# basilevh/occlusions-4d

Hardware: AMD Instinct MI355X
Metric: 4D query-points/sec (encode+decode) at n_points=14336 (higher is better)
Workload: dtype f32; 1 GPU; GREATER inference (BASELINE configs[1]): n_points=14336 video_len=12 num_sample=524288 (-> 534528 grid queries) implicit_batch_size=32768 (decoded in mini-batches of 32256 = 3584 workgroups of 9 queries; every query is decoded, results do not depend on the split), seeded random-init weights; abstract_points=531, outputs_per_query=5, parallelism=single GPU, schedule=sequential, rccl_ranks=1, decode_streams=2, decode_chunk=32256

## Files before the change

### occlusions-4d_amd/csrc/fps_bucket.hip

```cpp
#include "common.hpp"

#include <cstdlib>

namespace {

typedef unsigned long long u64;
typedef float f32x2 __attribute__((ext_vector_type(2)));

constexpr int FLAG_WORDS = 512;
constexpr int IDX_BITS = 14;
constexpr unsigned IDX_MASK = (1u << IDX_BITS) - 1u;

template <int OP>
__device__ __forceinline__ int wave_reduce(int v) {
#define OCC4D_DPP_STEP(ctrl)                                                                      \
  if (OP == 0) asm volatile("s_nop 1\n\tv_min_u32_dpp %0, %0, %0 " ctrl : "+v"(v));               \
  else asm volatile("s_nop 1\n\tv_max_i32_dpp %0, %0, %0 " ctrl : "+v"(v));
  OCC4D_DPP_STEP("quad_perm:[1,0,3,2] row_mask:0xf bank_mask:0xf")
  OCC4D_DPP_STEP("quad_perm:[2,3,0,1] row_mask:0xf bank_mask:0xf")
  OCC4D_DPP_STEP("row_half_mirror row_mask:0xf bank_mask:0xf")
  OCC4D_DPP_STEP("row_mirror row_mask:0xf bank_mask:0xf")
  OCC4D_DPP_STEP("row_bcast:15 row_mask:0xa bank_mask:0xf")
  OCC4D_DPP_STEP("row_bcast:31 row_mask:0xc bank_mask:0xf")
#undef OCC4D_DPP_STEP
  return __builtin_amdgcn_readlane(v, 63);
}

template <bool IS_MAX>
__device__ __forceinline__ float wave_reduce_f32(float v) {
#define OCC4D_DPP_STEP(ctrl)                                                                      \
  if (IS_MAX) asm volatile("s_nop 1\n\tv_max_f32_dpp %0, %0, %0 " ctrl : "+v"(v));               \
  else asm volatile("s_nop 1\n\tv_min_f32_dpp %0, %0, %0 " ctrl : "+v"(v));
  OCC4D_DPP_STEP("quad_perm:[1,0,3,2] row_mask:0xf bank_mask:0xf")
  OCC4D_DPP_STEP("quad_perm:[2,3,0,1] row_mask:0xf bank_mask:0xf")
  OCC4D_DPP_STEP("row_half_mirror row_mask:0xf bank_mask:0xf")
  OCC4D_DPP_STEP("row_mirror row_mask:0xf bank_mask:0xf")
  OCC4D_DPP_STEP("row_bcast:15 row_mask:0xa bank_mask:0xf")
  OCC4D_DPP_STEP("row_bcast:31 row_mask:0xc bank_mask:0xf")
#undef OCC4D_DPP_STEP
  return __int_as_float(__builtin_amdgcn_readlane(__float_as_int(v), 63));
}

template <typename E, int VL> struct vec_of { typedef E type __attribute__((ext_vector_type(VL))); };
constexpr int tuple_len(int len) { return len <= 2 ? 2 : len <= 4 ? 4 : len <= 8 ? 8 : len <= 16 ? 16 : 32; }

__device__ __forceinline__ unsigned spread3(unsigned x) {
  x = (x | (x << 8)) & 0x0300Fu;
  x = (x | (x << 4)) & 0x030C3u;
  x = (x | (x << 2)) & 0x09249u;
  return x;
}

__device__ __forceinline__ float block_reduce(float v, bool is_max, float* s_red, int t, int nw) {
  for (int o = 32; o > 0; o >>= 1) {
    const float w = __shfl_xor(v, o);
    v = is_max ? fmaxf(v, w) : fminf(v, w);
  }
  __syncthreads();
  if ((t & 63) == 0) s_red[t >> 6] = v;
  __syncthreads();
  float r = s_red[0];
  for (int w = 1; w < nw; ++w) r = is_max ? fmaxf(r, s_red[w]) : fminf(r, s_red[w]);
  return r;
}

template <int NB, int T>
__global__ __launch_bounds__(T) void fps_bucket_kernel(const float* __restrict__ xyz, int64_t stride, int n, int m,
                                                       int start, int32_t* __restrict__ out_sorted,
                                                       int32_t* __restrict__ out_order) {
  static_assert(NB >= 1 && NB <= 8, "buckets per wave: at most 8 (32 slots per lane)");
  constexpr int NW = T / 64;
  static_assert(NW == 8, "the candidate round below keeps candidate l % 8 in lane l");
  constexpr int CMAX = 8;
  constexpr int REFRESH = 8;
  constexpr int SORT_MAX = 16384;
  constexpr int CELL_BITS = 4, CELLS = 1 << (3 * CELL_BITS);
  static_assert(CELLS == 8 * T, "the scan below gives every thread eight cells");
  __shared__ unsigned short s_sort[SORT_MAX];
  __shared__ unsigned s_tmp[SORT_MAX];
  __shared__ unsigned s_hist[CELLS];
  __shared__ unsigned s_wsum[NW];
  __shared__ u64 s_key[2][NW];
  __shared__ float4 s_c[2][NW];
  __shared__ unsigned s_flags[FLAG_WORDS];
  __shared__ int s_cnt[T];
  __shared__ float s_red[NW];

  const int t = threadIdx.x;
  const int wave = t >> 6, lane = t & 63;

  float lo[3] = {__builtin_inff(), __builtin_inff(), __builtin_inff()};
  float hi[3] = {-__builtin_inff(), -__builtin_inff(), -__builtin_inff()};
  for (int i = t; i < n; i += T) {
    const float* p = xyz + (int64_t)i * stride;
#pragma unroll
    for (int a = 0; a < 3; ++a) {
      lo[a] = fminf(lo[a], p[a]);
      hi[a] = fmaxf(hi[a], p[a]);
    }
  }
  float scale[3];
#pragma unroll
  for (int a = 0; a < 3; ++a) {
    lo[a] = block_reduce(lo[a], false, s_red, t, NW);
    hi[a] = block_reduce(hi[a], true, s_red, t, NW);
    const float ext = hi[a] - lo[a];
    scale[a] = ext > 0.f ? (float)(1 << CELL_BITS) / ext : 0.f;
  }
  for (int c = t; c < CELLS; c += T) s_hist[c] = 0u;
  __syncthreads();
  for (int i = t; i < n; i += T) {
    const float* p = xyz + (int64_t)i * stride;
    unsigned cell = 0u;
#pragma unroll
    for (int a = 0; a < 3; ++a) {
      const int q = max(0, min((1 << CELL_BITS) - 1, (int)((p[a] - lo[a]) * scale[a])));
      cell |= spread3((unsigned)q) << a;
    }
    const unsigned rank = atomicAdd(&s_hist[cell], 1u);
    s_tmp[i] = (cell << IDX_BITS) | rank;
  }
  __syncthreads();
  {
    unsigned cnt[8], sum = 0u;
#pragma unroll
    for (int k = 0; k < 8; ++k) {
      cnt[k] = s_hist[8 * t + k];
      sum += cnt[k];
    }
    unsigned incl = sum;
    for (int o = 1; o < 64; o <<= 1) {
      const unsigned up = __shfl_up(incl, o);
      if (lane >= o) incl += up;
    }
    if (lane == 63) s_wsum[wave] = incl;
    __syncthreads();
    unsigned base = incl - sum;
    for (int w = 0; w < wave; ++w) base += s_wsum[w];
#pragma unroll
    for (int k = 0; k < 8; ++k) {
      s_hist[8 * t + k] = base;
      base += cnt[k];
    }
  }
  __syncthreads();
  for (int i = t; i < n; i += T) {
    const unsigned cr = s_tmp[i];
    s_sort[s_hist[cr >> IDX_BITS] + (cr & IDX_MASK)] = (unsigned short)i;
  }
  __syncthreads();

  constexpr int PPT = 4 * NB;
  typedef typename vec_of<float, tuple_len(PPT)>::type fvec;
  typedef typename vec_of<int, tuple_len(PPT)>::type ivec;
  typedef typename vec_of<int, tuple_len(2 * NB)>::type idvec;
  fvec px, py, pz;
  ivec md;
  idvec id;
  float bminx = 0.f, bminy = 0.f, bminz = 0.f, bmaxx = 0.f, bmaxy = 0.f, bmaxz = 0.f, bm = -1.f;
  const unsigned last = s_sort[n - 1];
#pragma clang loop unroll(disable)
  for (int u = 0; u < NB; ++u) {
    const int pos = ((u * NW + wave) << 8) + 4 * lane;
    float c[4][3], d0[4];
    unsigned ids[2] = {0u, 0u};
#pragma unroll
    for (int v = 0; v < 4; ++v) {
      const bool live = pos + v < n;
      const unsigned i = live ? (unsigned)s_sort[pos + v] : last;
      const float* p = xyz + (int64_t)i * stride;
      c[v][0] = p[0]; c[v][1] = p[1]; c[v][2] = p[2];
      d0[v] = live ? __builtin_inff() : -1.f;
      ids[v >> 1] |= (live ? i : 0xffffu) << (16 * (v & 1));
    }
    float bl[3], bh[3];
#pragma unroll
    for (int v = 0; v < 4; ++v) {
      px[4 * u + v] = c[v][0]; py[4 * u + v] = c[v][1]; pz[4 * u + v] = c[v][2];
      md[4 * u + v] = __float_as_int(d0[v]);
    }
    asm volatile("" : "+v"(ids[0]), "+v"(ids[1]));
    id[2 * u] = (int)ids[0]; id[2 * u + 1] = (int)ids[1];
#pragma unroll
    for (int a = 0; a < 3; ++a) {
      bl[a] = wave_reduce_f32<false>(fminf(fminf(c[0][a], c[1][a]), fminf(c[2][a], c[3][a])));
      bh[a] = wave_reduce_f32<true>(fmaxf(fmaxf(c[0][a], c[1][a]), fmaxf(c[2][a], c[3][a])));
    }
    const bool any_live = ((u * NW + wave) << 8) < n;
    if ((lane & 7) == u) {
      bminx = bl[0]; bminy = bl[1]; bminz = bl[2];
      bmaxx = bh[0]; bmaxy = bh[1]; bmaxz = bh[2];
      bm = any_live ? __builtin_inff() : -1.f;
    }
  }
  for (int w = t; w < FLAG_WORDS; w += T) s_flags[w] = 0u;
  __syncthreads();
  int gm[NB];
#pragma unroll
  for (int g = 0; g < NB; ++g) gm[g] = max(max(md[4 * g], md[4 * g + 1]), max(md[4 * g + 2], md[4 * g + 3]));
  const float* first = xyz + (int64_t)start * stride;
  float ccx = first[0], ccy = first[1], ccz = first[2];
  int nacc = 1;
  if (t == 0) {
    out_sorted[0] = start;
    if (out_order) out_order[0] = start;
  }

#ifdef OCC4D_FPSB_STAMP
  unsigned long long tacc[9] = {0, 0, 0, 0, 0, 0, 0, 0, 0};
  unsigned long long tprev = __builtin_amdgcn_s_memtime();
#define STAMP(i) { const unsigned long long tn = __builtin_amdgcn_s_memtime(); tacc[i] += tn - tprev; tprev = tn; }
#else
#define STAMP(i)
#endif
#define OCC4D_DPP8(op, v)                                                                          \
  asm volatile("s_nop 1\n\t" op " %0, %0, %0 quad_perm:[1,0,3,2] row_mask:0xf bank_mask:0xf\n\t"   \
               "s_nop 1\n\t" op " %0, %0, %0 quad_perm:[2,3,0,1] row_mask:0xf bank_mask:0xf\n\t"   \
               "s_nop 1\n\t" op " %0, %0, %0 row_half_mirror row_mask:0xf bank_mask:0xf" : "+v"(v))
  int par = 0, round = 0;
  for (int it = 1; it < m;) {
    if (round != 0 && (round & (REFRESH - 1)) == 0) {
#pragma unroll
      for (int u = 0; u < NB; ++u) {
        const int top = wave_reduce<1>(gm[u]);
        bm = (lane & 7) == u ? __int_as_float(top) : bm;
      }
    }
    ++round;
    const float ex = fmaxf(fmaxf(bminx - ccx, ccx - bmaxx), 0.f);
    const float ey = fmaxf(fmaxf(bminy - ccy, ccy - bmaxy), 0.f);
    const float ez = fmaxf(fmaxf(bminz - ccz, ccz - bmaxz), 0.f);
    const float db = (ex * ex + ey * ey) + ez * ez;
    const u64 touch = __ballot(db < bm && (lane >> 3) < nacc);
    STAMP(0)
#pragma unroll
    for (int u = 0; u < NB; ++u) {
      u64 mu = (touch >> u) & 0x0101010101010101ull;
      if (mu) {
        do {
          const int src = (int)__builtin_ctzll(mu) ;
          mu &= mu - 1;
          const float cx = __int_as_float(__builtin_amdgcn_readlane(__float_as_int(ccx), src));
          const float cy = __int_as_float(__builtin_amdgcn_readlane(__float_as_int(ccy), src));
          const float cz = __int_as_float(__builtin_amdgcn_readlane(__float_as_int(ccz), src));
          const f32x2 c2x = {cx, cx}, c2y = {cy, cy}, c2z = {cz, cz};
#pragma unroll
          for (int e = 4 * u; e < 4 * u + 4; e += 2) {
            const f32x2 dx = f32x2{px[e], px[e + 1]} - c2x;
            const f32x2 dy = f32x2{py[e], py[e + 1]} - c2y;
            const f32x2 dz = f32x2{pz[e], pz[e + 1]} - c2z;
            const f32x2 d = (dx * dx + dy * dy) + dz * dz;
            md[e] = min(__float_as_int(d[0]), md[e]);
            md[e + 1] = min(__float_as_int(d[1]), md[e + 1]);
          }
        } while (mu);
        gm[u] = max(max(md[4 * u], md[4 * u + 1]), max(md[4 * u + 2], md[4 * u + 3]));
      }
    }
    STAMP(1)
    int bd = gm[0];
#pragma unroll
    for (int g = 1; g < NB; ++g) bd = max(bd, gm[g]);
    const int wtop = wave_reduce<1>(bd);
    STAMP(2)
    constexpr int NEG1 = (int)0xbf800000;
    int hgroup = 0, lane_hits = 0, og = NEG1, sn = NEG1;
#pragma unroll
    for (int g = NB - 1; g >= 0; --g) {
      const bool e = gm[g] == wtop;
      hgroup = __ballot(e) ? g : hgroup;
      lane_hits += e ? 1 : 0;
      og = max(og, e ? NEG1 : gm[g]);
    }
    unsigned long long hit = 0ull;
    int hslot = 0, slot_hits = 0;
#pragma unroll
    for (int sl = 3; sl >= 0; --sl) {
      const int slot = hgroup * 4 + sl;
      const int v = md[slot];
      const bool e = v == wtop;
      const unsigned long long mk = __ballot(e);
      hit = mk ? mk : hit;
      hslot = mk ? slot : hslot;
      slot_hits += e ? 1 : 0;
      sn = max(sn, e ? NEG1 : v);
    }
    const bool single = __popcll(__ballot(lane_hits != 0)) == 1 && __ballot(lane_hits > 1 || slot_hits > 1) == 0ull;
    int hlane = (int)__builtin_ctzll(hit | (1ull << 63));
    unsigned widx;
    int wfloor = wtop;
    if (wtop >= 0 && !single) {
      unsigned cand = 0xffffffffu;
      int cslot = 0;
#pragma unroll
      for (int sl = 0; sl < PPT; ++sl) {
        const unsigned ids = (sl & 1) ? ((unsigned)id[sl >> 1] >> 16) : ((unsigned)id[sl >> 1] & 0xffffu);
        const bool better = md[sl] == wtop && ids < cand;
        cand = better ? ids : cand;
        cslot = better ? sl : cslot;
      }
      widx = (unsigned)wave_reduce<0>((int)cand);
      hlane = (int)__builtin_ctzll(__ballot(cand == widx) | (1ull << 63));
      hslot = __builtin_amdgcn_readlane(cslot, hlane);
    } else {
      const unsigned pair = (unsigned)__builtin_amdgcn_readlane(id[hslot >> 1], hlane);
      widx = (hslot & 1) ? (pair >> 16) : (pair & 0xffffu);
      if (wtop >= 0) wfloor = wave_reduce<1>(max(og, sn));
    }
    const float wx = __int_as_float(__builtin_amdgcn_readlane(__float_as_int(px[hslot]), hlane));
    const float wy = __int_as_float(__builtin_amdgcn_readlane(__float_as_int(py[hslot]), hlane));
    const float wz = __int_as_float(__builtin_amdgcn_readlane(__float_as_int(pz[hslot]), hlane));
    STAMP(3)
    if (lane == 0) {
      s_key[par][wave] = ((u64)(unsigned)max(wtop + 1, 0) << 32) |
                         (u64)(((IDX_MASK << 8) | (unsigned)wave) - ((widx & IDX_MASK) << 8));
      s_c[par][wave] = float4{wx, wy, wz, __int_as_float(wfloor)};
    }
    __syncthreads();
    STAMP(4)
    const int ci = lane & (NW - 1), ck = lane >> 3;
    const u64 key = s_key[par][ci];
    const float4 mine = s_c[par][ci], oth = s_c[par][ck];
    constexpr int TAKEN = (int)0x80000000, FAR = 0x7fffffff;
    const int khi = (int)(unsigned)(key >> 32);
    int cmd = khi ? khi - 1 : TAKEN;
    const int cidx = (int)(IDX_MASK - (((unsigned)key >> 8) & IDX_MASK));
    int fl = __float_as_int(mine.w);
    OCC4D_DPP8("v_max_i32_dpp", fl);
    const int F = __builtin_amdgcn_readfirstlane(fl);
    int D;
    {
      const float dx = mine.x - oth.x, dy = mine.y - oth.y, dz = mine.z - oth.z;
      D = __float_as_int((dx * dx + dy * dy) + dz * dz);
    }
    STAMP(5)
    const int room = min(CMAX, m - it);
    unsigned alist = 0u;
    int nnew = 0;
#pragma unroll
    for (int j = 0; j < CMAX; ++j) {
      int best = cmd;
      OCC4D_DPP8("v_max_i32_dpp", best);
      bool eq = cmd == best;
      unsigned m8 = (unsigned)__ballot(eq) & 0xffu;
      if (j == 0) {
        int low = eq ? cidx : FAR;
        OCC4D_DPP8("v_min_i32_dpp", low);
        eq = eq && cidx == low;
        m8 = (unsigned)__ballot(eq) & 0xffu;
      } else if (j >= room || !(__builtin_amdgcn_readfirstlane(best) > F) || (m8 & (m8 - 1u)) != 0u) {
        break;
      }
      const int a = __builtin_ctz(m8);
      alist |= (unsigned)a << (4 * j);
      nnew = j + 1;
      if (j == CMAX - 1) break;
      int red = ck == a ? D : FAR;
      asm volatile("s_nop 1\n\tv_min_i32_dpp %0, %0, %0 row_ror:8 row_mask:0xf bank_mask:0xf" : "+v"(red));
      {
        const auto r16 = __builtin_amdgcn_permlane16_swap((unsigned)red, (unsigned)red, false, false);
        red = min((int)r16[0], (int)r16[1]);
        const auto r32 = __builtin_amdgcn_permlane32_swap((unsigned)red, (unsigned)red, false, false);
        red = min((int)r32[0], (int)r32[1]);
      }
      cmd = eq ? TAKEN : min(cmd, red);
    }
    STAMP(6)
    {
      const int asel = (int)((alist >> (4 * ck)) & 7u);
      const float4 acc = s_c[par][asel];
      ccx = acc.x; ccy = acc.y; ccz = acc.z;
      if (wave == 0 && ci == 0 && ck < nnew) {
        const unsigned gi = IDX_MASK - (((unsigned)s_key[par][asel] >> 8) & IDX_MASK);
        const unsigned g = min(gi, (unsigned)(n - 1));
        out_sorted[it + ck] = (int)g;
        if (out_order) out_order[it + ck] = (int)g;
      }
    }
    nacc = nnew;
    it += nnew;
    STAMP(7)
    par ^= 1;
  }
#undef OCC4D_DPP8
  __syncthreads();
#ifdef OCC4D_FPSB_STAMP
  if (lane == 0 && out_order) {
    unsigned long long* o = (unsigned long long*)(out_order + ((m + 1) & ~1)) + wave * 16;
    tacc[8] = (unsigned long long)round;
#pragma unroll
    for (int i = 0; i < 9; ++i) o[i] = tacc[i];
  }
#endif

  for (int i = t; i < m; i += T) {
    const unsigned g = (unsigned)out_sorted[i];
    atomicOr(&s_flags[g >> 5], 1u << (g & 31));
  }
  __syncthreads();
  constexpr int CH = FLAG_WORDS / T;
  static_assert(CH >= 1, "T <= FLAG_WORDS");
  int cnt = 0;
#pragma unroll
  for (int c = 0; c < CH; ++c) cnt += __popc(s_flags[t * CH + c]);
  s_cnt[t] = cnt;
  __syncthreads();
  if (t == 0) {
    int run = 0;
    for (int i = 0; i < T; ++i) {
      const int c = s_cnt[i];
      s_cnt[i] = run;
      run += c;
    }
  }
  __syncthreads();
  int pos = s_cnt[t];
#pragma unroll
  for (int c = 0; c < CH; ++c) {
    unsigned wbits = s_flags[t * CH + c];
    while (wbits) {
      const int b = __ffs(wbits) - 1;
      wbits &= wbits - 1;
      if (pos < m) out_sorted[pos] = (t * CH + c) * 32 + b;
      ++pos;
    }
  }
}

}

namespace occ4d {

int fps_bucket_launch(const float* xyz, int64_t stride, int n, int m, int start, int32_t* os, int32_t* oo,
                      hipStream_t st) {
  static const int min_points = [] { const char* e = getenv("OCC4D_FPS_BUCKET_MIN"); return e ? atoi(e) : FPS_BUCKET_MIN_POINTS; }();
  if (n < min_points || n > 16384) return -1;
  constexpr int T = 512;
  const int nb = cdiv(n, 256 * (T / 64));
#define OCC4D_FPSB(B) fps_bucket_kernel<B, T><<<1, T, 0, st>>>(xyz, stride, n, m, start, os, oo)
  if (nb <= 1) OCC4D_FPSB(1);
  else if (nb <= 2) OCC4D_FPSB(2);
  else if (nb <= 3) OCC4D_FPSB(3);
  else if (nb <= 4) OCC4D_FPSB(4);
  else if (nb <= 5) OCC4D_FPSB(5);
  else if (nb <= 6) OCC4D_FPSB(6);
  else if (nb <= 7) OCC4D_FPSB(7);
  else OCC4D_FPSB(8);
#undef OCC4D_FPSB
  return 0;
}

}
```

Before: 4.651 million query-points/s.

## Propose two FPS candidates per wave to accept more points per round

Each wave in the bucketed farthest-point-sampling kernel now proposes its second-best point in addition to its best, giving 16 candidates per round. Wave 0 runs the greedy acceptance over all 16 with 16-lane DPP reductions and a 4-way distance table, then shares the accepted list through shared memory and an extra barrier. The aim is to accept more points per round and so cut the number of serial rounds and block-wide syncs. In exchange each round does more per-wave reduction work, adds a second __syncthreads, and leaves waves 1-7 idle during acceptance. The new path is the default, and OCC4D_FPS_CANDIDATES=1 restores the old one.

```diff
diff --git a/occlusions-4d_amd/csrc/fps_bucket.hip b/occlusions-4d_amd/csrc/fps_bucket.hip
--- a/occlusions-4d_amd/csrc/fps_bucket.hip
+++ b/occlusions-4d_amd/csrc/fps_bucket.hip
@@ -64,13 +64,15 @@
   return r;
 }
 
-template <int NB, int T>
+template <int NB, int T, int NC>
 __global__ __launch_bounds__(T) void fps_bucket_kernel(const float* __restrict__ xyz, int64_t stride, int n, int m,
                                                        int start, int32_t* __restrict__ out_sorted,
                                                        int32_t* __restrict__ out_order) {
   static_assert(NB >= 1 && NB <= 8, "buckets per wave: at most 8 (32 slots per lane)");
   constexpr int NW = T / 64;
-  static_assert(NW == 8, "the candidate round below keeps candidate l % 8 in lane l");
+  static_assert(NW == 8, "the candidate round below keeps candidate l % 8 (NC = 2: l % 16) in lane l");
+  static_assert(NC == 1 || NC == 2, "candidates per wave");
+  constexpr int NCAND = NC * NW;
   constexpr int CMAX = 8;
   constexpr int REFRESH = 8;
   constexpr int SORT_MAX = 16384;
@@ -80,8 +82,9 @@
   __shared__ unsigned s_tmp[SORT_MAX];
   __shared__ unsigned s_hist[CELLS];
   __shared__ unsigned s_wsum[NW];
-  __shared__ u64 s_key[2][NW];
-  __shared__ float4 s_c[2][NW];
+  __shared__ u64 s_key[2][NCAND];
+  __shared__ float4 s_c[2][NCAND];
+  __shared__ uint2 s_acc[2];
   __shared__ unsigned s_flags[FLAG_WORDS];
   __shared__ int s_cnt[T];
   __shared__ float s_red[NW];
@@ -217,6 +220,11 @@
   asm volatile("s_nop 1\n\t" op " %0, %0, %0 quad_perm:[1,0,3,2] row_mask:0xf bank_mask:0xf\n\t"   \
                "s_nop 1\n\t" op " %0, %0, %0 quad_perm:[2,3,0,1] row_mask:0xf bank_mask:0xf\n\t"   \
                "s_nop 1\n\t" op " %0, %0, %0 row_half_mirror row_mask:0xf bank_mask:0xf" : "+v"(v))
+#define OCC4D_DPP16(op, v)                                                                         \
+  asm volatile("s_nop 1\n\t" op " %0, %0, %0 quad_perm:[1,0,3,2] row_mask:0xf bank_mask:0xf\n\t"   \
+               "s_nop 1\n\t" op " %0, %0, %0 quad_perm:[2,3,0,1] row_mask:0xf bank_mask:0xf\n\t"   \
+               "s_nop 1\n\t" op " %0, %0, %0 row_half_mirror row_mask:0xf bank_mask:0xf\n\t"       \
+               "s_nop 1\n\t" op " %0, %0, %0 row_mirror row_mask:0xf bank_mask:0xf" : "+v"(v))
   int par = 0, round = 0;
   for (int it = 1; it < m;) {
     if (round != 0 && (round & (REFRESH - 1)) == 0) {
@@ -310,64 +318,169 @@
     const float wx = __int_as_float(__builtin_amdgcn_readlane(__float_as_int(px[hslot]), hlane));
     const float wy = __int_as_float(__builtin_amdgcn_readlane(__float_as_int(py[hslot]), hlane));
     const float wz = __int_as_float(__builtin_amdgcn_readlane(__float_as_int(pz[hslot]), hlane));
+    int w2 = NEG1;
+    unsigned widx2 = 0u;
+    float rx = 0.f, ry = 0.f, rz = 0.f;
+    if constexpr (NC == 2) {
+      if (single && wfloor >= 0) {
+        w2 = wfloor;
+        const bool wl = lane == hlane;
+        int hgroup2 = 0, group_hits2 = 0, og2 = NEG1, sn2 = NEG1;
+#pragma unroll
+        for (int g = NB - 1; g >= 0; --g) {
+          const int v = (wl && hgroup == g) ? sn : gm[g];
+          const bool e = v == w2;
+          const unsigned long long mk = __ballot(e);
+          hgroup2 = mk ? g : hgroup2;
+          group_hits2 += __popcll(mk);
+          og2 = max(og2, e ? NEG1 : v);
+        }
+        unsigned long long hit2 = 0ull;
+        int hslot2 = 0, slot_hits2 = 0;
+#pragma unroll
+        for (int sl = 3; sl >= 0; --sl) {
+          const int slot = hgroup2 * 4 + sl;
+          const int v = (wl && slot == hslot) ? NEG1 : md[slot];
+          const bool e = v == w2;
+          const unsigned long long mk = __ballot(e);
+          hit2 = mk ? mk : hit2;
+          hslot2 = mk ? slot : hslot2;
+          slot_hits2 += __popcll(mk);
+          sn2 = max(sn2, e ? NEG1 : v);
+        }
+        const bool single2 = group_hits2 == 1 && slot_hits2 == 1;
+        const int hlane2 = (int)__builtin_ctzll(hit2 | (1ull << 63));
+        const unsigned pair = (unsigned)__builtin_amdgcn_readlane(id[hslot2 >> 1], hlane2);
+        widx2 = (hslot2 & 1) ? (pair >> 16) : (pair & 0xffffu);
+        rx = __int_as_float(__builtin_amdgcn_readlane(__float_as_int(px[hslot2]), hlane2));
+        ry = __int_as_float(__builtin_amdgcn_readlane(__float_as_int(py[hslot2]), hlane2));
+        rz = __int_as_float(__builtin_amdgcn_readlane(__float_as_int(pz[hslot2]), hlane2));
+        if (single2) wfloor = wave_reduce<1>(max(og2, sn2));
+      }
+    }
     STAMP(3)
     if (lane == 0) {
-      s_key[par][wave] = ((u64)(unsigned)max(wtop + 1, 0) << 32) |
-                         (u64)(((IDX_MASK << 8) | (unsigned)wave) - ((widx & IDX_MASK) << 8));
-      s_c[par][wave] = float4{wx, wy, wz, __int_as_float(wfloor)};
+      s_key[par][NC * wave] = ((u64)(unsigned)max(wtop + 1, 0) << 32) |
+                              (u64)(((IDX_MASK << 8) | (unsigned)wave) - ((widx & IDX_MASK) << 8));
+      s_c[par][NC * wave] = float4{wx, wy, wz, __int_as_float(wfloor)};
+      if constexpr (NC == 2) {
+        s_key[par][2 * wave + 1] = ((u64)(unsigned)max(w2 + 1, 0) << 32) |
+                                   (u64)(((IDX_MASK << 8) | (unsigned)wave) - ((widx2 & IDX_MASK) << 8));
+        s_c[par][2 * wave + 1] = float4{rx, ry, rz, __int_as_float(wfloor)};
+      }
     }
     __syncthreads();
     STAMP(4)
     const int ci = lane & (NW - 1), ck = lane >> 3;
-    const u64 key = s_key[par][ci];
-    const float4 mine = s_c[par][ci], oth = s_c[par][ck];
     constexpr int TAKEN = (int)0x80000000, FAR = 0x7fffffff;
-    const int khi = (int)(unsigned)(key >> 32);
-    int cmd = khi ? khi - 1 : TAKEN;
-    const int cidx = (int)(IDX_MASK - (((unsigned)key >> 8) & IDX_MASK));
-    int fl = __float_as_int(mine.w);
-    OCC4D_DPP8("v_max_i32_dpp", fl);
-    const int F = __builtin_amdgcn_readfirstlane(fl);
-    int D;
-    {
-      const float dx = mine.x - oth.x, dy = mine.y - oth.y, dz = mine.z - oth.z;
-      D = __float_as_int((dx * dx + dy * dy) + dz * dz);
-    }
-    STAMP(5)
-    const int room = min(CMAX, m - it);
     unsigned alist = 0u;
     int nnew = 0;
-#pragma unroll
-    for (int j = 0; j < CMAX; ++j) {
-      int best = cmd;
-      OCC4D_DPP8("v_max_i32_dpp", best);
-      bool eq = cmd == best;
-      unsigned m8 = (unsigned)__ballot(eq) & 0xffu;
-      if (j == 0) {
-        int low = eq ? cidx : FAR;
-        OCC4D_DPP8("v_min_i32_dpp", low);
-        eq = eq && cidx == low;
-        m8 = (unsigned)__ballot(eq) & 0xffu;
-      } else if (j >= room || !(__builtin_amdgcn_readfirstlane(best) > F) || (m8 & (m8 - 1u)) != 0u) {
-        break;
-      }
-      const int a = __builtin_ctz(m8);
-      alist |= (unsigned)a << (4 * j);
-      nnew = j + 1;
-      if (j == CMAX - 1) break;
-      int red = ck == a ? D : FAR;
-      asm volatile("s_nop 1\n\tv_min_i32_dpp %0, %0, %0 row_ror:8 row_mask:0xf bank_mask:0xf" : "+v"(red));
+    if constexpr (NC == 1) {
+      const u64 key = s_key[par][ci];
+      const float4 mine = s_c[par][ci], oth = s_c[par][ck];
+      const int khi = (int)(unsigned)(key >> 32);
+      int cmd = khi ? khi - 1 : TAKEN;
+      const int cidx = (int)(IDX_MASK - (((unsigned)key >> 8) & IDX_MASK));
+      int fl = __float_as_int(mine.w);
+      OCC4D_DPP8("v_max_i32_dpp", fl);
+      const int F = __builtin_amdgcn_readfirstlane(fl);
+      int D;
       {
-        const auto r16 = __builtin_amdgcn_permlane16_swap((unsigned)red, (unsigned)red, false, false);
-        red = min((int)r16[0], (int)r16[1]);
-        const auto r32 = __builtin_amdgcn_permlane32_swap((unsigned)red, (unsigned)red, false, false);
-        red = min((int)r32[0], (int)r32[1]);
-      }
-      cmd = eq ? TAKEN : min(cmd, red);
+        const float dx = mine.x - oth.x, dy = mine.y - oth.y, dz = mine.z - oth.z;
+        D = __float_as_int((dx * dx + dy * dy) + dz * dz);
+      }
+      STAMP(5)
+      const int room = min(CMAX, m - it);
+#pragma unroll
+      for (int j = 0; j < CMAX; ++j) {
+        int best = cmd;
+        OCC4D_DPP8("v_max_i32_dpp", best);
+        bool eq = cmd == best;
+        unsigned m8 = (unsigned)__ballot(eq) & 0xffu;
+        if (j == 0) {
+          int low = eq ? cidx : FAR;
+          OCC4D_DPP8("v_min_i32_dpp", low);
+          eq = eq && cidx == low;
+          m8 = (unsigned)__ballot(eq) & 0xffu;
+        } else if (j >= room || !(__builtin_amdgcn_readfirstlane(best) > F) || (m8 & (m8 - 1u)) != 0u) {
+          break;
+        }
+        const int a = __builtin_ctz(m8);
+        alist |= (unsigned)a << (4 * j);
+        nnew = j + 1;
+        if (j == CMAX - 1) break;
+        int red = ck == a ? D : FAR;
+        asm volatile("s_nop 1\n\tv_min_i32_dpp %0, %0, %0 row_ror:8 row_mask:0xf bank_mask:0xf" : "+v"(red));
+        {
+          const auto r16 = __builtin_amdgcn_permlane16_swap((unsigned)red, (unsigned)red, false, false);
+          red = min((int)r16[0], (int)r16[1]);
+          const auto r32 = __builtin_amdgcn_permlane32_swap((unsigned)red, (unsigned)red, false, false);
+          red = min((int)r32[0], (int)r32[1]);
+        }
+        cmd = eq ? TAKEN : min(cmd, red);
+      }
+    } else {
+      const int cj = lane & (NCAND - 1), cq = lane >> 4;
+      if (wave == 0) {
+        const u64 key = s_key[par][cj];
+        const float4 mine = s_c[par][cj];
+        const int khi = (int)(unsigned)(key >> 32);
+        int cmd = khi ? khi - 1 : TAKEN;
+        const int cidx = (int)(IDX_MASK - (((unsigned)key >> 8) & IDX_MASK));
+        int fl = __float_as_int(mine.w);
+        OCC4D_DPP16("v_max_i32_dpp", fl);
+        const int F1 = __builtin_amdgcn_readfirstlane(fl) + 1;
+        int D[4];
+#pragma unroll
+        for (int r = 0; r < 4; ++r) {
+          const float4 oth = s_c[par][4 * cq + r];
+          const float dx = mine.x - oth.x, dy = mine.y - oth.y, dz = mine.z - oth.z;
+          D[r] = __float_as_int((dx * dx + dy * dy) + dz * dz);
+        }
+        STAMP(5)
+        const int room = min(CMAX, m - it);
+#pragma unroll
+        for (int j = 0; j < CMAX; ++j) {
+          int best = cmd;
+          OCC4D_DPP16("v_max_i32_dpp", best);
+          bool eq;
+          unsigned m16;
+          if (j == 0) {
+            eq = cmd == best;
+            int low = eq ? cidx : FAR;
+            OCC4D_DPP16("v_min_i32_dpp", low);
+            eq = eq && cidx == low;
+            m16 = (unsigned)__ballot(eq) & 0xffffu;
+          } else {
+            eq = cmd == max(best, F1);
+            m16 = (unsigned)__ballot(eq) & 0xffffu;
+            if (j >= room || __popc(m16) != 1) break;
+          }
+          const int a = __builtin_ctz(m16);
+          alist |= (unsigned)a << (4 * j);
+          nnew = j + 1;
+          if (j == CMAX - 1) break;
+          const int dlo = (a & 1) ? D[1] : D[0], dhi = (a & 1) ? D[3] : D[2];
+          const int dsel = (a & 2) ? dhi : dlo;
+          int red = cq == (a >> 2) ? dsel : FAR;
+          {
+            const auto r16 = __builtin_amdgcn_permlane16_swap((unsigned)red, (unsigned)red, false, false);
+            red = min((int)r16[0], (int)r16[1]);
+            const auto r32 = __builtin_amdgcn_permlane32_swap((unsigned)red, (unsigned)red, false, false);
+            red = min((int)r32[0], (int)r32[1]);
+          }
+          cmd = eq ? TAKEN : min(cmd, red);
+        }
+        if (lane == 0) s_acc[par] = uint2{alist, (unsigned)nnew};
+      }
+      __syncthreads();
+      const uint2 got = s_acc[par];
+      alist = (unsigned)__builtin_amdgcn_readfirstlane((int)got.x);
+      nnew = __builtin_amdgcn_readfirstlane((int)got.y);
     }
     STAMP(6)
     {
-      const int asel = (int)((alist >> (4 * ck)) & 7u);
+      const int asel = (int)((alist >> (4 * ck)) & (unsigned)(NCAND - 1));
       const float4 acc = s_c[par][asel];
       ccx = acc.x; ccy = acc.y; ccz = acc.z;
       if (wave == 0 && ci == 0 && ck < nnew) {
@@ -383,6 +496,7 @@
     par ^= 1;
   }
 #undef OCC4D_DPP8
+#undef OCC4D_DPP16
   __syncthreads();
 #ifdef OCC4D_FPSB_STAMP
   if (lane == 0 && out_order) {
@@ -434,10 +548,13 @@
 int fps_bucket_launch(const float* xyz, int64_t stride, int n, int m, int start, int32_t* os, int32_t* oo,
                       hipStream_t st) {
   static const int min_points = [] { const char* e = getenv("OCC4D_FPS_BUCKET_MIN"); return e ? atoi(e) : FPS_BUCKET_MIN_POINTS; }();
+  static const int candidates = [] { const char* e = getenv("OCC4D_FPS_CANDIDATES"); return e && atoi(e) == 1 ? 1 : 2; }();
   if (n < min_points || n > 16384) return -1;
   constexpr int T = 512;
   const int nb = cdiv(n, 256 * (T / 64));
-#define OCC4D_FPSB(B) fps_bucket_kernel<B, T><<<1, T, 0, st>>>(xyz, stride, n, m, start, os, oo)
+#define OCC4D_FPSB(B)                                                                                     \
+  if (candidates == 1) fps_bucket_kernel<B, T, 1><<<1, T, 0, st>>>(xyz, stride, n, m, start, os, oo);     \
+  else fps_bucket_kernel<B, T, 2><<<1, T, 0, st>>>(xyz, stride, n, m, start, os, oo)
   if (nb <= 1) OCC4D_FPSB(1);
   else if (nb <= 2) OCC4D_FPSB(2);
   else if (nb <= 3) OCC4D_FPSB(3);
```

Result: no change. 4.666 million query-points/s (median of 6 runs) (+0.3%).
